# jpreprocess/jbonsai

Hardware: AMD Instinct MI355X
Metric: 48 kHz PCM samples/sec (whole node), batched utterances (higher is better)
Workload: dtype f64

## Files before the change

### jbonsai_amd/csrc/jb_vocoder.hip

```cpp
#include "jb_device.h"

#include <cstdlib>
#include <cstring>

namespace jb {

__global__ void k_pitch(BatchDev bd, VocDev vd)
{
    const int b = blockIdx.y;
    const UttDev *u = bd.utt + b;
    const uint32_t t = blockIdx.x * blockDim.x + threadIdx.x;
    if (t >= u->T)
        return;
    const uint64_t f = u->frame_off + t;
    const double MAX_LF0 = 9.903487552536127, MIN_LF0 = 2.995732273553991;
    auto pitch_of = [&](double l) {
        if (l == kNoData)
            return 0.0;
        const double cl = l < MIN_LF0 ? MIN_LF0 : (l > MAX_LF0 ? MAX_LF0 : l);
        return (double)vd.fs / exp(cl);
    };
    const double p = pitch_of(vd.lf0[f]);
    const double prevp = t > 0 ? pitch_of(vd.lf0[f - 1]) : 0.0;
    vd.pitch[f] = p;
// ... 1157 lines not shown
                    yl = fma(cd[k], d[k], yl);
                const double Y = seg_scan(yl, ks);
                const double Yp = Y * Pl;
                const double v1 = readlane_f64(Yp, 11), v2 = readlane_f64(Yp, 23),
                             v3 = readlane_f64(Yp, 35), v4 = readlane_f64(Yp, 47),
                             v5 = readlane_f64(Yp, 59);
                x += v5;
                x -= v4;
                x += v3;
                x -= v2;
                x += v1;
                double out = v5;
                out += v4;
                out += v3;
                out += v2;
                out += v1;
                ulane = fma(hmask, dpp_f64<DPP_WAVE_SHR1>(Y), l0mask * x);
                x += out;
#pragma unroll
                for (int k = 0; k < TPL; k++)
                    cd[k] += cdinc[k];
                c1 += c1inc;
                ob = (lane == i) ? x * vol : ob;
            }
            if (lane < blen && emit) {
                if (vd.pcm16)
                    vd.pcm16[base * (uint64_t)fp + n0 + (uint64_t)lane] = (int16_t)pcm_i16(ob);
                else
                    vd.pcm[base * (uint64_t)fp + n0 + (uint64_t)lane] = ob;
            }
        }
        (void)ctgt;
    }

    if (wk.save_end)
        save_state(wk.save_end);
}

template <int TPL, int ITEMS>
__global__ __launch_bounds__(128 * ITEMS) void k_vocoder_pair(BatchDev bd, VocDev vd, const VocWork *__restrict__ work,
                                                              uint32_t n_items)
{
    __shared__ double xbuf[ITEMS][2][64];
    __shared__ double obuf[ITEMS][2][64];
    __shared__ uint32_t nblocks_sh[ITEMS];
    const int wv = threadIdx.x >> 6, lane = threadIdx.x & 63;
    const int slot = wv % ITEMS;
    const bool producer = wv >= ITEMS;
    const uint32_t item = blockIdx.x * (uint32_t)ITEMS + (uint32_t)slot;
    const int fp = vd.fperiod, bs = vd.bs, nblk = vd.nblk, nmcp = vd.nmcp;
    VocWork wk{};
    uint32_t t_begin = 0, t_end = 0, t_out = 0;
    int b = 0;
    if (item < n_items) {
        wk = work[item];
        b = (int)wk.utt;
        t_begin = wk.t_start;
        t_out = wk.t_out;
        t_end = min(wk.t_end, bd.utt[b].T);
        if (t_begin >= t_end)
            t_begin = t_end = 0;
    }
    const uint32_t NB = (t_end - t_begin) * (uint32_t)nblk;
    if (!producer && lane == 0)
        nblocks_sh[slot] = NB;
    __syncthreads();
    uint32_t NBmax = 0;
#pragma unroll
    for (int j = 0; j < ITEMS; j++)
        NBmax = max(NBmax, nblocks_sh[j]);
    const uint64_t base = NB ? bd.utt[b].frame_off : 0;
    const double a = wave_uniform(voc_alpha(vd, (uint32_t)b)), iaa = 1.0 - a * a,
                 vol = wave_uniform(voc_volume(vd, (uint32_t)b));
    double *const xb = &xbuf[slot][0][0];
    double *const ob = &obuf[slot][0][0];

    if (producer) {
        double e11[6], e12[6];
#pragma unroll
        for (int i = 0; i < 6; i++)
            e11[i] = e12[i] = 0.0;
        if (NB && wk.load_state) {
#pragma unroll
            for (int i = 0; i < 6; i++) {
                e11[i] = wk.load_state[64 * TPL + 64 + i];
                e12[i] = wk.load_state[64 * TPL + 70 + i];
            }
        }
        auto save_state = [&](double *sp) {
            if (lane == 0) {
#pragma unroll
                for (int i = 0; i < 6; i++) {
                    sp[64 * TPL + 64 + i] = e11[i];
                    sp[64 * TPL + 70 + i] = e12[i];
                }
            }
        };
        uint32_t t = t_begin;
        int q = 0;
        double c1 = 0.0, c1inc = 0.0, gain = 0.0, gq = 0.0;
        for (uint32_t st = 0; st < NBmax + 2; st++) {
            if (st >= 2 && st - 2 < NB) {
                const uint32_t gb = st - 2;
                const uint32_t ts = t_begin + gb / (uint32_t)nblk;
                const int qs = (int)(gb % (uint32_t)nblk), i0 = qs * bs;
                const int blen = min(bs, fp - i0);
                if (ts >= t_out && lane < blen) {
                    const double v = ob[64 * (gb & 1u) + lane] * vol;
                    const uint64_t o = base * (uint64_t)fp + (uint64_t)ts * (uint64_t)fp + (uint64_t)(i0 + lane);
                    if (vd.pcm16)
                        vd.pcm16[o] = (int16_t)pcm_i16(v);
                    else
                        vd.pcm[o] = v;
                }
            }
            if (st < NB) {
                if (q == 0) {
                    if (t == t_out && t_out > t_begin && wk.save_warm)
                        save_state(wk.save_warm);
                    if (t == t_out + vd.ckpt_frames && wk.save_ckpt)
                        save_state(wk.save_ckpt);
                    if (vd.ckpt2_frames && t == t_out + vd.ckpt2_frames && wk.save_ckpt2)
                        save_state(wk.save_ckpt2);
                    const double *bcur = vd.bcoef + (base + t) * (uint64_t)nmcp;
                    const double *bprev =
                        (t > 0) ? bcur - nmcp : (vd.bfirst ? vd.bfirst + (uint64_t)b * (uint64_t)nmcp : bcur);
                    c1 = bprev[1];
                    c1inc = (bcur[1] - c1) / (double)fp;
                    gain = exp(bprev[0]);
                    gq = exp((bcur[0] - bprev[0]) / (double)fp);
                }
                const int i0 = q * bs;
                const int blen = min(bs, fp - i0);
                const double xin = lane < blen ? exc_block_ptr(vd, base, t, exc_code(vd, base, t), q)[i0 + lane] : 0.0;
                double xo = 0.0;
                for (int i = 0; i < blen; i++) {
                    double x = readlane_f64(xin, i) * gain;
                    gain *= gq;
                    double out = 0.0;
#pragma unroll
                    for (int ii = 5; ii >= 1; ii--) {
                        e11[ii] = fma(iaa, e12[ii - 1], a * e11[ii]);
                        e12[ii] = e11[ii] * c1;
                        const double v = e12[ii] * kPPade[ii];
                        x += (ii & 1) ? v : -v;
                        out += v;
                    }
                    e12[0] = x;
                    x += out;
                    c1 += c1inc;
                    xo = (lane == i) ? x : xo;
                }
                if (lane < blen)
                    xb[64 * (st & 1u) + lane] = xo;
                if (++q == nblk) {
                    q = 0;
                    t++;
                }
            }
            __syncthreads();
        }
        if (NB && wk.save_end)
            save_state(wk.save_end);
        return;
    }

    const int M = nmcp - 1;
    const int s = lane / kGroups, g = lane % kGroups;
    const bool active = lane < kPade * kGroups;
    const bool head = active && g == 0;
    const double kappa = ipow(-a, TPL);
    ScanCoef kc, ks;
    {
        const int r16 = lane & 15;
        auto ok = [&](int sh) { return active && g >= sh && r16 >= sh; };
        kc.c1 = ok(1) ? ipow(kappa, 1) : 0.0;
        kc.c2 = ok(2) ? ipow(kappa, 2) : 0.0;
        kc.c4 = ok(4) ? ipow(kappa, 4) : 0.0;
        kc.c8 = ok(8) ? ipow(kappa, 8) : 0.0;
        const int rowstart = lane & ~15, segstart = s * kGroups;
        const bool straddle = active && rowstart > 0 && segstart < rowstart;
        kc.cb = straddle ? ipow(kappa, lane - rowstart + 1) : 0.0;
        ks.c1 = kc.c1 != 0.0 ? 1.0 : 0.0;
        ks.c2 = kc.c2 != 0.0 ? 1.0 : 0.0;
        ks.c4 = kc.c4 != 0.0 ? 1.0 : 0.0;
        ks.c8 = kc.c8 != 0.0 ? 1.0 : 0.0;
        ks.cb = straddle ? 1.0 : 0.0;
    }
    const double nh = (active && !head) ? 1.0 : 0.0;
    const double hmask = (head && s > 0) ? 1.0 : 0.0;
    const double l0mask = (lane == 0) ? 1.0 : 0.0;
    const double Pl = active ? kPPade[s + 1] : 0.0;
    int tapj[TPL];
    bool dotv[TPL];
#pragma unroll
    for (int k = 0; k < TPL; k++) {
        tapj[k] = g * TPL + k + 1;
        dotv[k] = active && tapj[k] >= 2 && tapj[k] <= M;
    }
    double d[TPL], cd[TPL], cdinc[TPL];
#pragma unroll
    for (int k = 0; k < TPL; k++)
        d[k] = cd[k] = cdinc[k] = 0.0;
    double ulane = 0.0;
    if (NB && wk.load_state) {
#pragma unroll
        for (int k = 0; k < TPL; k++)
            d[k] = wk.load_state[64 * k + lane];
        ulane = wk.load_state[64 * TPL + lane];
    }
    auto save_state = [&](double *sp) {
#pragma unroll
        for (int k = 0; k < TPL; k++)
            sp[64 * k + lane] = d[k];
        sp[64 * TPL + lane] = ulane;
    };
    uint32_t t = t_begin;
    int q = 0;
    for (uint32_t st = 0; st < NBmax + 2; st++) {
        if (st >= 1 && st - 1 < NB) {
            const uint32_t gb = st - 1;
            if (q == 0) {
                if (t == t_out && t_out > t_begin && wk.save_warm)
                    save_state(wk.save_warm);
                if (t == t_out + vd.ckpt_frames && wk.save_ckpt)
                    save_state(wk.save_ckpt);
                if (vd.ckpt2_frames && t == t_out + vd.ckpt2_frames && wk.save_ckpt2)
                    save_state(wk.save_ckpt2);
                const double *bcur = vd.bcoef + (base + t) * (uint64_t)nmcp;
                const double *bprev = (t > 0) ? bcur - nmcp : (vd.bfirst ? vd.bfirst + (uint64_t)b * (uint64_t)nmcp : bcur);
#pragma unroll
                for (int k = 0; k < TPL; k++) {
                    const double c0v = dotv[k] ? bprev[tapj[k]] : 0.0;
                    const double c1v = dotv[k] ? bcur[tapj[k]] : 0.0;
                    cd[k] = c0v;
                    cdinc[k] = (c1v - c0v) / (double)fp;
                }
            }
            const int blen = min(bs, fp - q * bs);
            const double *xs = xb + 64 * (gb & 1u);
            double *os = ob + 64 * (gb & 1u);
            double xn = xs[0];
            for (int i = 0; i < blen; i++) {
                double x = xn;
                xn = xs[i + 1 < blen ? i + 1 : i];
                double loc = d[0];
#pragma unroll
                for (int k = 1; k < TPL; k++)
                    loc = fma(-a, loc, d[k]);
                double I = fma(kappa, ulane, loc);
                I = seg_scan(I, kc);
                double r = fma(nh, dpp_f64<DPP_WAVE_SHR1>(I), ulane);
#pragma unroll
                for (int k = 0; k < TPL; k++) {
                    const double rn = fma(-a, r, d[k]);
                    d[k] = fma(a, rn, r);
                    r = rn;
                }
                double yl = cd[0] * d[0];
#pragma unroll
                for (int k = 1; k < TPL; k++)
                    yl = fma(cd[k], d[k], yl);
                const double Y = seg_scan(yl, ks);
                const double Yp = Y * Pl;
                const double v1 = readlane_f64(Yp, 11), v2 = readlane_f64(Yp, 23), v3 = readlane_f64(Yp, 35),
                             v4 = readlane_f64(Yp, 47), v5 = readlane_f64(Yp, 59);
                x += v5;
                x -= v4;
                x += v3;
                x -= v2;
                x += v1;
                double out = v5;
                out += v4;
                out += v3;
                out += v2;
                out += v1;
                ulane = fma(hmask, dpp_f64<DPP_WAVE_SHR1>(Y), l0mask * x);
                x += out;
#pragma unroll
                for (int k = 0; k < TPL; k++)
                    cd[k] += cdinc[k];
                if (lane == 0)
                    os[i] = x;
            }
            if (++q == nblk) {
                q = 0;
                t++;
            }
        }
        __syncthreads();
    }
    if (NB && wk.save_end)
        save_state(wk.save_end);
}

constexpr int DPP_WAVE_SHL1 = 0x130;
constexpr int DPP_ROW_SHL1 = 0x101, DPP_ROW_SHL2 = 0x102, DPP_ROW_SHL4 = 0x104;
__device__ __forceinline__ double fold5(double s)
{
    const double t1 = s + dpp_f64<DPP_ROW_SHL1>(s);
    const double t2 = t1 + dpp_f64<DPP_ROW_SHL2>(t1);
    return t2 + dpp_f64<DPP_ROW_SHL4>(s);
}
constexpr int kLtPf = 4;
constexpr int kLtBalance = 8;
#ifdef JB_LT_STAMPS
constexpr unsigned kLtStampWaves = 4096;
__device__ unsigned long long g_lt_stamp[kLtStampWaves][4];
#endif
#ifdef JB_LT_CLOCKS
__device__ unsigned long long g_lt_clk[8];
#endif

template <int NM, int TPLW_, int kLtWaves, bool EXACT = true, int LPC = 3>
__global__ __launch_bounds__(64 * kLtWaves, 2) void k_vocoder_lt(BatchDev bd, VocDev vd,
                                                       const VocWork *__restrict__ work,
                                                       const uint32_t *__restrict__ order,
                                                       uint32_t n_items)
{
    static_assert(LPC == 3 || LPC == 5, "three lanes x two stage slots, or five lanes x one");
    constexpr int M = NM - 1;
    constexpr int NS = LPC == 3 ? 2 : 1;
    constexpr int kLtChunks = lt_chunks(LPC);
    const int nm = EXACT ? NM : vd.nmcp;
    const int mreal = nm - 1;
    const int TPLW = EXACT ? TPLW_ : (mreal + kGroups - 1) / kGroups;
    const int lane = threadIdx.x % 64;
    const int wv = threadIdx.x / 64;
    const bool idle = LPC == 3 ? lane == 63 : (lane & 15) == 15;
    const int pos = LPC == 3 ? (idle ? 2 : lane % 3) : (idle ? 4 : (lane & 15) % 5);
    const int ci = LPC == 3 ? (idle ? 20 : lane / 3) : (lane >> 4) * 3 + (idle ? 2 : (lane & 15) / 5);
    const uint32_t slot = (blockIdx.x * (uint32_t)kLtWaves + (uint32_t)wv) * (uint32_t)kLtChunks + (uint32_t)ci;
    const uint32_t oslot = (!idle && slot < n_items) ? order[slot] : kLtNoItem;
    const bool has = oslot != kLtNoItem;
    const bool lead = has && pos == 0;
    const uint32_t item = has ? oslot : 0u;
    struct {
        uint32_t utt, t_start, t_out, t_end;
        const double *load_state;
    } wk = {0, 0, 0, 0, nullptr};
    if (has) {
        const VocWork &w0 = work[item];
        wk.utt = w0.utt;
        wk.t_start = w0.t_start;
        wk.t_out = w0.t_out;
        wk.t_end = w0.t_end;
        wk.load_state = w0.load_state;
    }
    const uint32_t T = has ? bd.utt[wk.utt].T : 0;
    if (wk.t_end > T)
        wk.t_end = T;
    const uint32_t nfr = wk.t_end > wk.t_start ? wk.t_end - wk.t_start : 0;
    uint32_t maxfr = nfr;
    for (int o = 32; o > 0; o >>= 1)
        maxfr = max(maxfr, (uint32_t)__shfl_xor((int)maxfr, o));
    __shared__ uint32_t prog[8];
    if (kLtWaves == 8 && lane == 0)
        prog[wv] = maxfr == 0 ? 0xffffffffu : 0u;
    if (maxfr == 0)
        return;
#ifdef JB_LT_STAMPS
    const unsigned stamp_w = blockIdx.x * (unsigned)kLtWaves + (unsigned)wv;
    if (lane == 0 && stamp_w < kLtStampWaves) {
        unsigned hw, xcc;
        asm volatile("s_getreg_b32 %0, hwreg(HW_REG_HW_ID)" : "=s"(hw));
        asm volatile("s_getreg_b32 %0, hwreg(HW_REG_XCC_ID, 0, 4)" : "=s"(xcc));
        g_lt_stamp[stamp_w][0] = wall_clock64();
        g_lt_stamp[stamp_w][2] = (unsigned long long)hw | ((unsigned long long)xcc << 32);
        g_lt_stamp[stamp_w][3] = maxfr;
    }
#endif
#ifdef JB_LT_CLOCKS
    const int clk_slot = wv != 0 ? -1 : blockIdx.x == 0 ? 0 : blockIdx.x == gridDim.x / 2 ? 4 : -1;
    if (clk_slot >= 0 && lane == 0) {
        g_lt_clk[clk_slot] = clock64();
        g_lt_clk[clk_slot + 1] = wall_clock64();
    }
#endif
    const uint64_t base = has ? bd.utt[wk.utt].frame_off : 0;
    const int fp = vd.fperiod;
    double a = vd.alpha, vol = vd.volume;
    if (vd.uvoc) {
        const uint32_t u0 = wave_uniform(wk.utt);
        a = wave_uniform(vd.uvoc[u0].alpha);
        vol = wave_uniform(vd.uvoc[u0].volume);
    }
    const double na = -a, iaa = 1.0 - a * a;
    const int s0 = NS * pos;
    const double w0 = kPPade[s0 + 1];
    const double w1 = (NS == 2 && s0 + 1 < kPade) ? kPPade[s0 + 2] : 0.0;
    const double wa = (NS == 1 && (pos & 1)) ? -w0 : w0;

    __shared__ double2 cc_[kLtWaves][NM - 1][kLtChunks];
    __shared__ double gqs_[kLtWaves][kLtChunks];
    double2 (*const cc)[kLtChunks] = cc_[wv];
    double *const gqs = gqs_[wv];
#define JB_LT_FENCE() asm volatile("s_waitcnt lgkmcnt(0)" ::: "memory")

    if (!EXACT && has)
        for (int k = nm + pos; k < NM; k += LPC)
            cc[k - 1][ci] = make_double2(0.0, 0.0);
    double d[NS][M + 1];
    double u[NS];
    double gain = 1.0;
    double e11[NS], e12[NS], ein = 0.0;
#pragma unroll
    for (int q = 0; q < NS; q++) {
        e11[q] = e12[q] = 0.0;
        u[q] = 0.0;
#pragma unroll
        for (int j = 0; j <= M; j++)
            d[q][j] = 0.0;
    }

    auto layout_tpl = [&]() {
        int tp = TPLW;
        if (!EXACT)
            asm volatile("" : "+s"(tp));
        return tp;
    };
    if (wk.load_state) {
        const double *sp = wk.load_state;
        const int tpl = layout_tpl();
#pragma unroll
        for (int q = 0; q < NS; q++) {
            const int st = s0 + q;
            if (st < kPade) {
                u[q] = sp[64 * tpl + kGroups * st];
                int kk = 0, gg = 0;
#pragma unroll
                for (int j = 1; j <= M; j++) {
                    if (EXACT)
                        d[q][j] = sp[64 * ((j - 1) % TPLW_) + kGroups * st + (j - 1) / TPLW_];
                    else if (j <= mreal)
                        d[q][j] = sp[64 * kk + kGroups * st + gg];
                    if (++kk == tpl) {
                        kk = 0;
                        gg++;
                    }
                }
            }
        }
#pragma unroll
        for (int q = 0; q < NS; q++) {
            const int st = s0 + 1 + q;
            if (st <= kPade) {
                e11[q] = sp[64 * tpl + 64 + st];
                e12[q] = sp[64 * tpl + 70 + st];
            }
        }
        ein = sp[64 * tpl + 70 + s0];
    }
    auto save_state = [&](double *sp) {
        const int tpl = layout_tpl();
#pragma unroll
        for (int q = 0; q < NS; q++) {
            const int st = s0 + q;
            if (st < kPade) {
                sp[64 * tpl + kGroups * st] = u[q];
                int kk = 0, gg = 0;
#pragma unroll
                for (int j = 1; j <= M; j++) {
                    if (EXACT)
                        sp[64 * ((j - 1) % TPLW_) + kGroups * st + (j - 1) / TPLW_] = d[q][j];
                    else if (j <= mreal)
                        sp[64 * kk + kGroups * st + gg] = d[q][j];
                    if (++kk == tpl) {
                        kk = 0;
                        gg++;
                    }
                }
            }
        }
#pragma unroll
        for (int q = 0; q < NS; q++) {
            const int st = s0 + 1 + q;
            if (st <= kPade) {
                sp[64 * tpl + 64 + st] = e11[q];
                sp[64 * tpl + 70 + st] = e12[q];
            }
        }
        if (pos == 0) {
            sp[64 * tpl + 64] = 0.0;
            sp[64 * tpl + 70] = ein;
        }
    };

    for (uint32_t tl = 0; tl < maxfr; tl++) {
        const bool act = tl < nfr;
        const uint32_t t = wk.t_start + (act ? tl : 0);
        const uint64_t f = base + t;
        const bool emit = act && lead && t >= wk.t_out;
        if (act && t == wk.t_out && wk.t_out > wk.t_start) {
            double *sw_ = work[item].save_warm;
            if (sw_)
                save_state(sw_);
        }
        if (act && t == wk.t_out + vd.ckpt_frames) {
            double *sc_ = work[item].save_ckpt;
            if (sc_)
                save_state(sc_);
        }
        if (act && vd.ckpt2_frames && t == wk.t_out + vd.ckpt2_frames) {
            double *sc_ = work[item].save_ckpt2;
            if (sc_)
                save_state(sc_);
        }
        JB_LT_FENCE();
        if (has) {
            const double *bcur = vd.bcoef + f * (uint64_t)nm;
            const double *bprev = (t > 0) ? bcur - nm : (vd.bfirst ? vd.bfirst + (uint64_t)wk.utt * nm : bcur);
            for (int k = 1 + pos; k < nm; k += LPC) {
                const double c0v = bprev[k], c1v = bcur[k];
                cc[k - 1][ci] = make_double2(c0v, (c1v - c0v) / (double)fp);
            }
            gain = exp(bprev[0]);
            if (pos == 0)
                gqs[ci] = exp((bcur[0] - bprev[0]) / (double)fp);
        }
        JB_LT_FENCE();
        const uint32_t xcode = act ? exc_code(vd, base, t) : 1u;
        const int xbs = vd.bs;
        auto xblock = [&](int q) -> const double * { return act ? exc_block_ptr(vd, base, t, xcode, q) : vd.noise; };
        const double *xq = xblock(0);
        double *op = vd.pcm + (base + t) * (uint64_t)fp;
        double xn = act ? xq[0] : 0.0;
        const double gq = gqs[ci];
        double oA = 0.0, oB = 0.0;
        auto put_pair = [&](int at) {
            if (vd.pcm16)
                *reinterpret_cast<uint32_t *>(vd.pcm16 + (base + t) * (uint64_t)fp + at) = pcm_i16x2(oA, oB);
            else
                *reinterpret_cast<double2 *>(op + at) = make_double2(oA, oB);
        };
        double xo;
        {
            const int n1 = fp > 1 ? 1 : 0;
            asm volatile("global_load_dwordx2 %0, %1, off" : "=v"(xo) : "v"(xq + n1) : "memory");
        }
        auto sample = [&](const int i, auto ODDC) {
            constexpr bool ODD = decltype(ODDC)::value;
            double x;
            if (ODD) {
                asm volatile("s_waitcnt vmcnt(0)" : "+v"(xo)::"memory");
                x = xo * gain;
            } else {
                asm volatile("s_waitcnt vmcnt(1)" : "+v"(xn)::"memory");
                x = xn * gain;
            }
            gain *= gq;
            if (!ODD && i > 0 && emit)
                put_pair(i - 2);
            {
                const int nx = i + 2 < fp ? i + 2 : fp - 1;
                if (ODD)
                    asm volatile("global_load_dwordx2 %0, %1, off" : "=v"(xo) : "v"(xq + nx) : "memory");
                else
                    asm volatile("global_load_dwordx2 %0, %1, off" : "=v"(xn) : "v"(xq + nx) : "memory");
            }
            const double fi = (double)i;
            double db1;
            {
                const double2 c1p = cc[0][ci];
                const double c1 = fma(fi, c1p.y, c1p.x);
                if constexpr (NS == 2) {
                    e11[1] = fma(iaa, e12[0], a * e11[1]);
                    e11[0] = fma(iaa, ein, a * e11[0]);
                    e12[1] = e11[1] * c1;
                    e12[0] = e11[0] * c1;
                    const double dv1 = w1 * e12[1];
                    const double da = fma(w0, e12[0], -dv1);
                    db1 = fma(w0, e12[0], dv1);
                    x += da + dpp_f64<DPP_WAVE_SHL1>(da + dpp_f64<DPP_WAVE_SHL1>(da));
                } else {
                    e11[0] = fma(iaa, ein, a * e11[0]);
                    e12[0] = e11[0] * c1;
                    db1 = w0 * e12[0];
                    x += fold5(wa * e12[0]);
                }
                const double eprev = dpp_f64<DPP_WAVE_SHR1>(e12[NS - 1]);
                ein = pos == 0 ? x : eprev;
            }
            double r[NS], y[NS];
#pragma unroll
            for (int q = 0; q < NS; q++)
                r[q] = u[q];
            static_assert(M >= 2, "the dot products start at tap 2");
            typedef double v2d __attribute__((ext_vector_type(2)));
            v2d cq[kLtPf];
            const uint32_t cca = (uint32_t)(uintptr_t)&cc[0][ci];
#define JB_LDS_RD(dst, tapj)                                                                     \
    asm volatile("ds_read_b128 %0, %1 offset:%2"                                                 \
                 : "=v"(dst)                                                                     \
                 : "v"(cca), "n"(((tapj)-1) * (int)(sizeof(double2) * kLtChunks)))
#pragma unroll
            for (int k = 0; k < kLtPf; k++)
                JB_LDS_RD(cq[k], 2 + k);
            static_assert(kLtPf == 4 && M % 2 == 0 && M >= 6, "pair schedule: four slots, taps 2..M in pairs + one");
            double cv[M + 2];
            auto wait_pair = [&](const int j, const int younger) {
                v2d &qa = cq[(j - 2) % kLtPf], &qb = cq[(j - 1) % kLtPf];
                switch (younger) {
                case 0: asm volatile("s_waitcnt lgkmcnt(0)" : "+v"(qa), "+v"(qb)); break;
                case 1: asm volatile("s_waitcnt lgkmcnt(1)" : "+v"(qa), "+v"(qb)); break;
                default: asm volatile("s_waitcnt lgkmcnt(2)" : "+v"(qa), "+v"(qb)); break;
                }
            };
            cv[1] = 0.0;
#pragma unroll
            for (int j = 1; j <= M; j++) {
                if (j == 1)
                    wait_pair(2, 2);
                else if (j % 2 == 0 && j + 2 <= M)
                    wait_pair(j + 2, j + 4 <= M ? 1 : 0);
                if (j + 1 <= M) {
                    const int sq = (j - 1) % kLtPf;
                    cv[j + 1] = fma(fi, cq[sq].y, cq[sq].x);
                    if (j + 5 <= M)
                        JB_LDS_RD(cq[sq], j + 5);
                }
                const double cj = cv[j];
                if constexpr (NS == 1) {
                    double rn0;
                    if (j <= 2) {
                        asm volatile("v_fma_f64 %[rn0], %[na], %[r0], %[d0]\n\t"
                            "v_fma_f64 %[d0], %[a], %[rn0], %[r0]"
                            : [rn0] "=&v"(rn0), [d0] "+v"(d[0][j])
                            : [na] "s"(na), [a] "s"(a), [r0] "v"(r[0]));
                    } else if (j == 3) {
                        asm volatile("v_fma_f64 %[rn0], %[na], %[r0], %[d0]\n\t"
                            "v_mul_f64 %[y0], %[c], %[dp]\n\t"
                            "v_fma_f64 %[d0], %[a], %[rn0], %[r0]"
                            : [rn0] "=&v"(rn0), [d0] "+v"(d[0][j]), [y0] "=&v"(y[0])
                            : [na] "s"(na), [a] "s"(a), [r0] "v"(r[0]), [c] "v"(cv[j - 1]), [dp] "v"(d[0][j - 1]));
                    } else {
                        asm volatile("v_fma_f64 %[rn0], %[na], %[r0], %[d0]\n\t"
                            "v_fma_f64 %[y0], %[c], %[dp], %[y0]\n\t"
                            "v_fma_f64 %[d0], %[a], %[rn0], %[r0]"
                            : [rn0] "=&v"(rn0), [d0] "+v"(d[0][j]), [y0] "+v"(y[0])
                            : [na] "s"(na), [a] "s"(a), [r0] "v"(r[0]), [c] "v"(cv[j - 1]), [dp] "v"(d[0][j - 1]));
                    }
                    r[0] = rn0;
                    if (j == M)
                        y[0] = fma(cj, d[0][M], y[0]);
                } else {
                    double rn0, rn1;
                    if (j == 2) {
                        asm volatile("v_fma_f64 %[rn0], %[na], %[r0], %[d0]\n\t"
                            "v_fma_f64 %[rn1], %[na], %[r1], %[d1]\n\t"
                            "v_fma_f64 %[d0], %[a], %[rn0], %[r0]\n\t"
                            "v_fma_f64 %[d1], %[a], %[rn1], %[r1]\n\t"
                            "v_mul_f64 %[y0], %[c], %[d0]\n\t"
                            "v_mul_f64 %[y1], %[c], %[d1]"
                            : [rn0] "=&v"(rn0), [rn1] "=&v"(rn1), [d0] "+v"(d[0][j]), [d1] "+v"(d[1][j]),
                              [y0] "=&v"(y[0]), [y1] "=&v"(y[1])
                            : [na] "s"(na), [a] "s"(a), [r0] "v"(r[0]), [r1] "v"(r[1]), [c] "v"(cj));
                    } else if (j > 2) {
                        asm volatile("v_fma_f64 %[rn0], %[na], %[r0], %[d0]\n\t"
                            "v_fma_f64 %[rn1], %[na], %[r1], %[d1]\n\t"
                            "v_fma_f64 %[d0], %[a], %[rn0], %[r0]\n\t"
                            "v_fma_f64 %[d1], %[a], %[rn1], %[r1]\n\t"
                            "v_fma_f64 %[y0], %[c], %[d0], %[y0]\n\t"
                            "v_fma_f64 %[y1], %[c], %[d1], %[y1]"
                            : [rn0] "=&v"(rn0), [rn1] "=&v"(rn1), [d0] "+v"(d[0][j]), [d1] "+v"(d[1][j]),
                              [y0] "+v"(y[0]), [y1] "+v"(y[1])
                            : [na] "s"(na), [a] "s"(a), [r0] "v"(r[0]), [r1] "v"(r[1]), [c] "v"(cj));
                    } else {
                        asm volatile("v_fma_f64 %[rn0], %[na], %[r0], %[d0]\n\t"
                            "v_fma_f64 %[rn1], %[na], %[r1], %[d1]\n\t"
                            "v_fma_f64 %[d0], %[a], %[rn0], %[r0]\n\t"
                            "v_fma_f64 %[d1], %[a], %[rn1], %[r1]"
                            : [rn0] "=&v"(rn0), [rn1] "=&v"(rn1), [d0] "+v"(d[0][j]), [d1] "+v"(d[1][j])
                            : [na] "s"(na), [a] "s"(a), [r0] "v"(r[0]), [r1] "v"(r[1]));
                    }
                    r[0] = rn0;
                    r[1] = rn1;
                }
            }
#undef JB_LDS_RD
            double ssum, psum;
            if constexpr (NS == 2) {
                const double v1 = w1 * y[1];
                const double sb = fma(w0, y[0], v1), sa = fma(w0, y[0], db1 - v1);
                ssum = sa + dpp_f64<DPP_WAVE_SHL1>(sa + dpp_f64<DPP_WAVE_SHL1>(sa));
                psum = sb + dpp_f64<DPP_WAVE_SHL1>(sb + dpp_f64<DPP_WAVE_SHL1>(sb));
            } else {
                ssum = fold5(fma(wa, y[0], db1));
                psum = fold5(w0 * y[0]);
            }
            const double yprev = dpp_f64<DPP_WAVE_SHR1>(y[NS - 1]);
            const double xmid = x + ssum;
            x = xmid + psum;
            if constexpr (NS == 2)
                u[1] = y[0];
            u[0] = pos == 0 ? xmid : yprev;
            const double pv = x * vol;
            if (ODD)
                oB = pv;
            else
                oA = pv;
        };
        int xnext = xbs, xqn = 1;
        for (int i2 = 0; i2 < fp; i2 += 2) {
            if (i2 + 2 == xnext && xnext < fp) {
                xq = xblock(xqn);
                xqn++;
                xnext += xbs;
            }
            if (kLtWaves == 8 && i2 % kLtBalance == 0) {
                const uint32_t mine = tl * (uint32_t)fp + (uint32_t)i2;
                uint32_t theirs;
                asm volatile("ds_write_b32 %1, %2\n\t"
                             "ds_read_b32 %0, %3\n\t"
                             "s_waitcnt lgkmcnt(0)"
                             : "=v"(theirs)
                             : "v"((uint32_t)(uintptr_t)&prog[wv]), "v"(mine), "v"((uint32_t)(uintptr_t)&prog[wv ^ 4])
                             : "memory");
                if (mine > (uint32_t)__builtin_amdgcn_readfirstlane((int)theirs))
                    __builtin_amdgcn_s_setprio(0);
                else
                    __builtin_amdgcn_s_setprio(1);
            }
            sample(i2, std::false_type{});
            sample(i2 + 1, std::true_type{});
        }
        asm volatile("s_waitcnt vmcnt(0)" : "+v"(xn), "+v"(xo)::"memory");
        if (emit)
            put_pair(fp - 2);
        if (act && tl + 1 == nfr) {
            double *se_ = work[item].save_end;
            if (se_)
                save_state(se_);
        }
    }
    if (kLtWaves == 8 && lane == 0)
        prog[wv] = 0xffffffffu;
#ifdef JB_LT_STAMPS
    if (lane == 0 && stamp_w < kLtStampWaves)
        g_lt_stamp[stamp_w][1] = wall_clock64();
#endif
#ifdef JB_LT_CLOCKS
    if (clk_slot >= 0 && lane == 0) {
        g_lt_clk[clk_slot + 2] = clock64();
        g_lt_clk[clk_slot + 3] = wall_clock64();
    }
#endif
}

__device__ __forceinline__ bool voc_state_differs(const double *__restrict__ a, const double *__restrict__ r,
                                                  int nfilt, int ntaps, double tol, int lane, double *md_out,
                                                  double *mr_out)
{
    double md = 0.0, mr = 0.0;
    const int urow = nfilt - 76;
    const int tpl = urow / 64;
    for (int k = lane; k < nfilt; k += 64) {
        if (ntaps < 0) {
        } else if (k < urow) {
            const int ln = k & 63, kk = k >> 6;
            if (ln >= kGroups * kPade || (ln % kGroups) * tpl + kk >= ntaps)
                continue;
        } else if (k < urow + 64 && ((k - urow) % kGroups != 0 || (k - urow) >= kGroups * kPade)) {
            continue;
        }
        const double x = a[k], y = r[k];
        md = fmax(md, fabs(x - y));
        mr = fmax(mr, fabs(y));
        if (!(x == x) || !(y == y))
            md = 1e300;
    }
    for (int o = 32; o > 0; o >>= 1) {
        md = fmax(md, __shfl_xor(md, o));
        mr = fmax(mr, __shfl_xor(mr, o));
    }
    *md_out = md;
    *mr_out = mr;
    return md > tol * mr && md > 1e-300;
}

__global__ __launch_bounds__(64) void k_voc_verify(const VocWork *__restrict__ work, uint32_t n_items,
                                                    int nfilt , int ntaps, double tol,
                                                    uint8_t *bad, uint32_t *n_bad)
{
    const uint32_t i = blockIdx.x;
    if (i >= n_items)
        return;
    const VocWork wk = work[i];
    const int lane = threadIdx.x;
    if (!wk.save_warm || i == 0) {
        if (lane == 0)
            bad[i] = 0;
        return;
    }
    double md, mr;
    const bool isbad = voc_state_differs(wk.save_warm, work[i - 1].save_end, nfilt, ntaps, tol, lane, &md, &mr);
    if (lane == 0) {
        bad[i] = isbad;
        if (isbad)
            atomicAdd(n_bad, 1u);
#ifdef JB_VERIFY_DEBUG
        if (isbad)
            printf("handoff item %u utt %u t_out %u: max|diff| %.3e max|state| %.3e ratio %.3e\n", i, wk.utt,
                   wk.t_out, md, mr, md / mr);
#endif
    }
}

__global__ __launch_bounds__(64) void k_voc_verify_pairs(const double *const *__restrict__ pairs, uint32_t n_pairs,
                                                          int nfilt, int ntaps, double tol, uint8_t *bad,
                                                          uint32_t *n_bad)
{
    const uint32_t i = blockIdx.x;
    if (i >= n_pairs)
        return;
    const int lane = threadIdx.x;
    double md, mr;
    const bool isbad = voc_state_differs(pairs[2 * i], pairs[2 * i + 1], nfilt, ntaps, tol, lane, &md, &mr);
    if (lane == 0) {
        bad[i] = isbad;
        if (isbad)
            atomicAdd(n_bad, 1u);
#ifdef JB_VERIFY_DEBUG
        printf("state pair %u: max|diff| %.3e max|state| %.3e %s\n", i, md, mr, isbad ? "FAIL" : "ok");
#endif
    }
}

static int tpl_for(int nmcp)
{
    int M = nmcp - 1;
    int tpl = (M + kGroups - 1) / kGroups;
    return tpl < 1 ? 1 : tpl;
}

int vocoder_state_doubles(int nmcp) { return voc_state_doubles(tpl_for(nmcp)); }

hipError_t launch_pitch(const BatchDev &bd, const VocDev &vd, hipStream_t stream)
{
    if (bd.B == 0 || bd.maxT == 0)
        return hipSuccess;
    dim3 grid((bd.maxT + 255) / 256, bd.B), block(256);
    hipLaunchKernelGGL(k_pitch, grid, block, 0, stream, bd, vd);
    return hipGetLastError();
}

hipError_t launch_mc2b(const BatchDev &bd, const VocDev &vd, hipStream_t stream)
{
    if (bd.B == 0 || bd.maxT == 0)
        return hipSuccess;
    dim3 grid((bd.maxT + kMc2bFrames - 1) / kMc2bFrames, bd.B), block(kMc2bFrames);
    hipLaunchKernelGGL(k_mc2b, grid, block, 0, stream, bd, vd);
    return hipGetLastError();
}

static int current_device_cus()
{
    static int cus_of[64] = {0};
    int dev = 0, cus = 0;
    if (hipGetDevice(&dev) != hipSuccess || dev < 0 || dev >= 64)
        return 0;
    if ((cus = cus_of[dev]) == 0) {
        if (hipDeviceGetAttribute(&cus, hipDeviceAttributeMultiprocessorCount, dev) != hipSuccess || cus <= 0)
            return 0;
        cus_of[dev] = cus;
    }
    return cus;
}

bool excite_is_split(const VocDev &vd)
{
    return vd.fperiod % kExw == 0 && vd.fperiod <= 256 && vd.fperiod >= kExwHalo && (vd.nlpf == 31 || vd.nlpf == 15) &&
           vd.nblk <= 4 && vd.fperiod % vd.bs == 0;
}

hipError_t launch_excite_noise(const BatchDev &bd, const VocDev &vd, hipStream_t stream)
{
    if (bd.B == 0 || bd.maxT == 0 || !excite_is_split(vd))
        return hipSuccess;
    if (!vd.exc_src || !vd.exc_gen || !vd.exc_gen_count || !vd.exc_tab)
        return hipErrorInvalidValue;
    hipError_t e = hipMemsetAsync(vd.exc_gen_count, 0, sizeof(uint32_t), stream);
    if (e != hipSuccess)
        return e;
    const dim3 block(256);
    const dim3 gcls((bd.maxT + 255) / 256, bd.B), gtab((bd.maxT + 3) / 4);
    constexpr size_t pad = 32 * 1024;
    int cus = current_device_cus();
    if (cus <= 0)
        cus = 256;
    const dim3 ggen((unsigned)(3 * cus));
    if (vd.nlpf == 31) {
        hipLaunchKernelGGL(k_exc_classify<31>, gcls, block, 0, stream, bd, vd);
        if (!vd.exc_no_table)
            hipLaunchKernelGGL(k_exc_table<31>, gtab, block, 0, stream, bd, vd);
        JB_DBG_SKIP_IF(4, hipLaunchKernelGGL(k_exc_general<31>, ggen, block, pad, stream, bd, vd));
    } else {
        hipLaunchKernelGGL(k_exc_classify<15>, gcls, block, 0, stream, bd, vd);
        if (!vd.exc_no_table)
            hipLaunchKernelGGL(k_exc_table<15>, gtab, block, 0, stream, bd, vd);
        hipLaunchKernelGGL(k_exc_general<15>, ggen, block, pad, stream, bd, vd);
    }
    return hipGetLastError();
}

hipError_t launch_excite(const BatchDev &bd, const VocDev &vd, hipStream_t stream)
{
    if (bd.B == 0 || bd.maxT == 0)
        return hipSuccess;
    if (excite_is_split(vd)) {
        dim3 gfix((bd.maxT + 4 * kFixFrames - 1) / (4 * kFixFrames), bd.B), block(256);
        if (vd.nlpf == 31)
            JB_DBG_SKIP_IF(8, hipLaunchKernelGGL(k_excite_fix<31>, gfix, block, 0, stream, bd, vd));
        else
            hipLaunchKernelGGL(k_excite_fix<15>, gfix, block, 0, stream, bd, vd);
        return hipGetLastError();
    }
    const uint64_t maxN = (uint64_t)bd.maxT * (uint64_t)vd.fperiod;
    dim3 grid((unsigned)((maxN + kExcBlock - 1) / kExcBlock), bd.B), block(kExcBlock);
    if (vd.nlpf == 0) {
        if (!vd.uv_before)
            return hipErrorInvalidValue;
        hipLaunchKernelGGL(k_uv_scan, dim3(bd.B), dim3(64), 0, stream, bd, vd);
        hipLaunchKernelGGL(k_excite_nolpf, grid, block, 0, stream, bd, vd);
        return hipGetLastError();
    }
    if (excite_fits_staged(vd))
        hipLaunchKernelGGL(k_excite, grid, block, 0, stream, bd, vd);
    else
        hipLaunchKernelGGL(k_excite_any, grid, block, (size_t)(kExcBlock + vd.nlpf - 1) * sizeof(double), stream, bd, vd);
    return hipGetLastError();
}

constexpr unsigned kPulseQueueWaves = 512;
hipError_t launch_pulse(const BatchDev &bd, const VocDev &vd, hipStream_t stream)
{
    if (bd.B == 0 || bd.maxT == 0)
        return hipSuccess;
    hipLaunchKernelGGL(k_run_scan, dim3(1), dim3(256), 0, stream, bd, vd);
    JB_DBG_SKIP_IF(64, hipLaunchKernelGGL(k_pulse_queue, dim3(kPulseQueueWaves), dim3(64), 0, stream, bd, vd));
    return hipGetLastError();
}

hipError_t launch_voc_verify(const VocWork *work_dev, uint32_t n_items, int state_doubles, int ntaps, double tol,
                             uint8_t *bad, uint32_t *n_bad, hipStream_t stream)
{
    if (n_items == 0)
        return hipSuccess;
    hipLaunchKernelGGL(k_voc_verify, dim3(n_items), dim3(64), 0, stream, work_dev, n_items,
                       ntaps < 0 ? state_doubles : state_doubles - 4, ntaps, tol, bad, n_bad);
    return hipGetLastError();
}

hipError_t launch_voc_verify_pairs(const double *const *pairs_dev, uint32_t n_pairs, int state_doubles, int ntaps,
                                   double tol, uint8_t *bad, uint32_t *n_bad, hipStream_t stream)
{
    if (n_pairs == 0)
        return hipSuccess;
    hipLaunchKernelGGL(k_voc_verify_pairs, dim3(n_pairs), dim3(64), 0, stream, pairs_dev, n_pairs,
                       ntaps < 0 ? state_doubles : state_doubles - 4, ntaps, tol, bad, n_bad);
    return hipGetLastError();
}

hipError_t launch_vocoder_ls(const BatchDev &bd, const VocDev &vd, const VocWork *work_dev,
                             const uint32_t *order_dev, uint32_t n_items, int waves_per_simd, hipStream_t stream)
{
    if (n_items == 0)
        return hipSuccess;
    if ((waves_per_simd != 1 && waves_per_simd != 2) || !vocoder_ls_supported(vd.nmcp))
        return hipErrorInvalidValue;
    const int wv = 4 * waves_per_simd;
    const int code = lt_code_nm(vd.nmcp);
    const bool exact = vd.nmcp == 35 || vd.nmcp == 25;
    const uint32_t per_wg = (uint32_t)(vocoder_ls_chunks_per_wave(vd.nmcp) * wv);
    dim3 grid((n_items + per_wg - 1) / per_wg), block(64 * wv);
#define JB_LT_LAUNCH(NMc, TPLc, EX, LPCc)                                                                              \
    do {                                                                                                           \
        if (wv == 8)                                                                                               \
            hipLaunchKernelGGL((k_vocoder_lt<NMc, TPLc, 8, EX, LPCc>), grid, block, 0, stream, bd, vd, work_dev,      \
                               order_dev, n_items);                                                                \
        else                                                                                                       \
            hipLaunchKernelGGL((k_vocoder_lt<NMc, TPLc, 4, EX, LPCc>), grid, block, 0, stream, bd, vd, work_dev,      \
                               order_dev, n_items);                                                                \
    } while (0)
    if (exact && code == 35)
        JB_LT_LAUNCH(35, 3, true, 3);
    else if (exact && code == 25)
        JB_LT_LAUNCH(25, 2, true, 3);
    else if (code == 25)
        JB_LT_LAUNCH(25, 2, false, 3);
    else if (code == 31)
        JB_LT_LAUNCH(31, 3, false, 3);
    else if (code == 35)
        JB_LT_LAUNCH(35, 3, false, 3);
    else if (code == 41)
        JB_LT_LAUNCH(41, 4, false, 5);
    else if (code == 51)
        JB_LT_LAUNCH(51, 5, false, 5);
    else
        JB_LT_LAUNCH(61, 5, false, 5);
#undef JB_LT_LAUNCH
#ifdef JB_LT_STAMPS
    if (const char *path = getenv("JB_LT_STAMPS_FILE")) {
        static unsigned long long st[kLtStampWaves][4];
        hipStreamSynchronize(stream);
        const unsigned nw = std::min<unsigned>(kLtStampWaves, grid.x * (unsigned)wv);
        if (hipMemcpyFromSymbol(st, HIP_SYMBOL(g_lt_stamp), sizeof st) == hipSuccess)
            if (FILE *f = fopen(path, "w")) {
                fprintf(f, "# wave start_10ns end_10ns hw_id xcc frames   (k_vocoder_lt, %u waves, %d per workgroup)\n", nw, wv);
                for (unsigned w = 0; w < nw; w++)
                    fprintf(f, "%u %llu %llu %llu %llu %llu\n", w, st[w][0], st[w][1], st[w][2] & 0xffffffffull,
                            st[w][2] >> 32, st[w][3]);
                fclose(f);
            }
        unsigned long long t0 = ~0ull, last[16] = {0};
        for (unsigned w = 0; w < nw; w++)
            if (st[w][0] && st[w][0] < t0)
                t0 = st[w][0];
        for (unsigned w = 0; w < nw; w++)
            last[(st[w][2] >> 32) & 15] = std::max(last[(st[w][2] >> 32) & 15], st[w][1]);
        fprintf(stderr, "k_vocoder_lt last wave end per XCD, ms:");
        for (int x = 0; x < 8; x++)
            fprintf(stderr, " %.2f", last[x] ? (double)(last[x] - t0) / 1e5 : 0.0);
        fprintf(stderr, "\n");
    }
#endif
#ifdef JB_LT_CLOCKS
    {
        unsigned long long c[8];
        hipStreamSynchronize(stream);
        if (hipMemcpyFromSymbol(c, HIP_SYMBOL(g_lt_clk), sizeof c) == hipSuccess)
            for (int k = 0; k < 8; k += 4) {
                const double us = (double)(c[k + 3] - c[k + 1]) / 100.0;
                fprintf(stderr, "k_vocoder_lt wave %d: %.3f ms, %.0f shader-clock ticks = %.3f GHz\n", k / 4, us / 1e3,
                        (double)(c[k + 2] - c[k]), (double)(c[k + 2] - c[k]) / us / 1e3);
            }
    }
#endif
// ... 78 lines not shown
```

Baseline: 20.26 billion.

## Defer cross-lane output reductions via ds_bpermute to overlap with next sample

For the two-stage-per-lane layout, the cross-lane shifts for the input-side sum, the post-filter sum and the previous-lane state are moved from DPP to asynchronous ds_bpermute LDS ops. The final output combine is deferred into the next sample, where it is waited on alongside other LDS reads, so the latency sits off the serial dependency chain. The output pointer is also advanced incrementally instead of being recomputed per pair. The risk is more LDS traffic and extra register pressure from the carried partial values, plus subtle ordering hazards in the pipelined recurrence.

```diff
diff --git a/jbonsai_amd/csrc/jb_vocoder.hip b/jbonsai_amd/csrc/jb_vocoder.hip
--- a/jbonsai_amd/csrc/jb_vocoder.hip
+++ b/jbonsai_amd/csrc/jb_vocoder.hip
@@ -1483,6 +1483,10 @@
     const double t2 = t1 + dpp_f64<DPP_ROW_SHL2>(t1);
     return t2 + dpp_f64<DPP_ROW_SHL4>(s);
 }
+struct LtXd {
+    int lo, hi;
+};
+__device__ __forceinline__ double lt_xd(const LtXd &v) { return __hiloint2double(v.hi, v.lo); }
 constexpr int kLtPf = 4;
 constexpr int kLtBalance = 8;
 #ifdef JB_LT_STAMPS
@@ -1632,6 +1636,11 @@
         }
         ein = sp[64 * tpl + 70 + s0];
     }
+    [[maybe_unused]] const uint32_t bpa = (uint32_t)lane * 4u;
+#define JB_BPERM(dst, src, off) \
+    asm volatile("ds_bpermute_b32 %0, %1, %2 offset:%3" : "=v"(dst) : "v"(bpa), "v"(src), "n"(off))
+    [[maybe_unused]] double xmid_c = u[0], sb_c = 0.0;
+    [[maybe_unused]] LtXd yp_c = {__double2loint(u[0]), __double2hiint(u[0])}, p1_c = {0, 0}, p2_c = {0, 0};
     auto save_state = [&](double *sp) {
         const int tpl = layout_tpl();
 #pragma unroll
@@ -1704,23 +1713,35 @@
         const int xbs = vd.bs;
         auto xblock = [&](int q) -> const double * { return act ? exc_block_ptr(vd, base, t, xcode, q) : vd.noise; };
         const double *xq = xblock(0);
-        double *op = vd.pcm + (base + t) * (uint64_t)fp;
+        const int64_t pstep = vd.pcm16 ? 4 : 16;
+        char *pq = vd.pcm16 ? reinterpret_cast<char *>(vd.pcm16 + (base + t) * (uint64_t)fp)
+                            : reinterpret_cast<char *>(vd.pcm + (base + t) * (uint64_t)fp);
         double xn = act ? xq[0] : 0.0;
         const double gq = gqs[ci];
         double oA = 0.0, oB = 0.0;
-        auto put_pair = [&](int at) {
+        auto put_pair = [&](auto BACK) {
+            constexpr int back = decltype(BACK)::value;
             if (vd.pcm16)
-                *reinterpret_cast<uint32_t *>(vd.pcm16 + (base + t) * (uint64_t)fp + at) = pcm_i16x2(oA, oB);
+                *reinterpret_cast<uint32_t *>(pq - back * 4) = pcm_i16x2(oA, oB);
             else
-                *reinterpret_cast<double2 *>(op + at) = make_double2(oA, oB);
+                *reinterpret_cast<double2 *>(pq - back * 16) = make_double2(oA, oB);
         };
         double xo;
         {
             const int n1 = fp > 1 ? 1 : 0;
             asm volatile("global_load_dwordx2 %0, %1, off" : "=v"(xo) : "v"(xq + n1) : "memory");
         }
+        typedef double v2d __attribute__((ext_vector_type(2)));
+        const uint32_t cca = (uint32_t)(uintptr_t)&cc[0][ci];
+        [[maybe_unused]] auto collect = [&](double &o) {
+            u[0] = pos == 0 ? xmid_c : lt_xd(yp_c);
+            o = (xmid_c + (sb_c + (lt_xd(p1_c) + lt_xd(p2_c)))) * vol;
+        };
         auto sample = [&](const int i, auto ODDC) {
             constexpr bool ODD = decltype(ODDC)::value;
+            v2d c1q;
+            if constexpr (NS == 2)
+                asm volatile("ds_read_b128 %0, %1" : "=v"(c1q) : "v"(cca));
             double x;
             if (ODD) {
                 asm volatile("s_waitcnt vmcnt(0)" : "+v"(xo)::"memory");
@@ -1730,8 +1751,17 @@
                 x = xn * gain;
             }
             gain *= gq;
-            if (!ODD && i > 0 && emit)
-                put_pair(i - 2);
+            if constexpr (NS == 2) {
+                asm volatile("s_waitcnt lgkmcnt(0)"
+                             : "+v"(c1q), "+v"(yp_c.lo), "+v"(yp_c.hi), "+v"(p1_c.lo), "+v"(p1_c.hi), "+v"(p2_c.lo),
+                               "+v"(p2_c.hi));
+                collect(ODD ? oA : oB);
+            }
+            if (!ODD) {
+                pq += pstep;
+                if (i > 0 && emit)
+                    put_pair(std::integral_constant<int, 2>{});
+            }
             {
                 const int nx = i + 2 < fp ? i + 2 : fp - 1;
                 if (ODD)
@@ -1741,25 +1771,33 @@
             }
             const double fi = (double)i;
             double db1;
-            {
+            [[maybe_unused]] double da;
+            [[maybe_unused]] LtXd d1, d2, ep;
+            if constexpr (NS == 2) {
+                const double c1 = fma(fi, c1q.y, c1q.x);
+                e11[1] = fma(iaa, e12[0], a * e11[1]);
+                e11[0] = fma(iaa, ein, a * e11[0]);
+                e12[1] = e11[1] * c1;
+                e12[0] = e11[0] * c1;
+                const double dv1 = w1 * e12[1];
+                da = fma(w0, e12[0], -dv1);
+                db1 = fma(w0, e12[0], dv1);
+                const int dal = __double2loint(da), dah = __double2hiint(da);
+                const int epl = __double2loint(e12[1]), eph = __double2hiint(e12[1]);
+                JB_BPERM(d1.lo, dal, 4);
+                JB_BPERM(d1.hi, dah, 4);
+                JB_BPERM(d2.lo, dal, 8);
+                JB_BPERM(d2.hi, dah, 8);
+                JB_BPERM(ep.lo, epl, 252);
+                JB_BPERM(ep.hi, eph, 252);
+            } else {
                 const double2 c1p = cc[0][ci];
                 const double c1 = fma(fi, c1p.y, c1p.x);
-                if constexpr (NS == 2) {
-                    e11[1] = fma(iaa, e12[0], a * e11[1]);
-                    e11[0] = fma(iaa, ein, a * e11[0]);
-                    e12[1] = e11[1] * c1;
-                    e12[0] = e11[0] * c1;
-                    const double dv1 = w1 * e12[1];
-                    const double da = fma(w0, e12[0], -dv1);
-                    db1 = fma(w0, e12[0], dv1);
-                    x += da + dpp_f64<DPP_WAVE_SHL1>(da + dpp_f64<DPP_WAVE_SHL1>(da));
-                } else {
-                    e11[0] = fma(iaa, ein, a * e11[0]);
-                    e12[0] = e11[0] * c1;
-                    db1 = w0 * e12[0];
-                    x += fold5(wa * e12[0]);
-                }
-                const double eprev = dpp_f64<DPP_WAVE_SHR1>(e12[NS - 1]);
+                e11[0] = fma(iaa, ein, a * e11[0]);
+                e12[0] = e11[0] * c1;
+                db1 = w0 * e12[0];
+                x += fold5(wa * e12[0]);
+                const double eprev = dpp_f64<DPP_WAVE_SHR1>(e12[0]);
                 ein = pos == 0 ? x : eprev;
             }
             double r[NS], y[NS];
@@ -1767,9 +1805,7 @@
             for (int q = 0; q < NS; q++)
                 r[q] = u[q];
             static_assert(M >= 2, "the dot products start at tap 2");
-            typedef double v2d __attribute__((ext_vector_type(2)));
             v2d cq[kLtPf];
-            const uint32_t cca = (uint32_t)(uintptr_t)&cc[0][ci];
 #define JB_LDS_RD(dst, tapj)                                                                     \
     asm volatile("ds_read_b128 %0, %1 offset:%2"                                                 \
                  : "=v"(dst)                                                                     \
@@ -1790,9 +1826,17 @@
             cv[1] = 0.0;
 #pragma unroll
             for (int j = 1; j <= M; j++) {
-                if (j == 1)
-                    wait_pair(2, 2);
-                else if (j % 2 == 0 && j + 2 <= M)
+                if (j == 1) {
+                    if constexpr (NS == 2) {
+                        asm volatile("s_waitcnt lgkmcnt(2)"
+                                     : "+v"(cq[0]), "+v"(cq[1]), "+v"(d1.lo), "+v"(d1.hi), "+v"(d2.lo), "+v"(d2.hi),
+                                       "+v"(ep.lo), "+v"(ep.hi));
+                        x += da + (lt_xd(d1) + lt_xd(d2));
+                        ein = pos == 0 ? x : lt_xd(ep);
+                    } else {
+                        wait_pair(2, 2);
+                    }
+                } else if (j % 2 == 0 && j + 2 <= M)
                     wait_pair(j + 2, j + 4 <= M ? 1 : 0);
                 if (j + 1 <= M) {
                     const int sq = (j - 1) % kLtPf;
@@ -1859,27 +1903,34 @@
                 }
             }
 #undef JB_LDS_RD
-            double ssum, psum;
             if constexpr (NS == 2) {
                 const double v1 = w1 * y[1];
                 const double sb = fma(w0, y[0], v1), sa = fma(w0, y[0], db1 - v1);
-                ssum = sa + dpp_f64<DPP_WAVE_SHL1>(sa + dpp_f64<DPP_WAVE_SHL1>(sa));
-                psum = sb + dpp_f64<DPP_WAVE_SHL1>(sb + dpp_f64<DPP_WAVE_SHL1>(sb));
+                const double ssum = sa + dpp_f64<DPP_WAVE_SHL1>(sa + dpp_f64<DPP_WAVE_SHL1>(sa));
+                const int sbl = __double2loint(sb), sbh = __double2hiint(sb);
+                const int ypl = __double2loint(y[1]), yph = __double2hiint(y[1]);
+                JB_BPERM(p1_c.lo, sbl, 4);
+                JB_BPERM(p1_c.hi, sbh, 4);
+                JB_BPERM(p2_c.lo, sbl, 8);
+                JB_BPERM(p2_c.hi, sbh, 8);
+                JB_BPERM(yp_c.lo, ypl, 252);
+                JB_BPERM(yp_c.hi, yph, 252);
+                xmid_c = x + ssum;
+                sb_c = sb;
+                u[1] = y[0];
             } else {
-                ssum = fold5(fma(wa, y[0], db1));
-                psum = fold5(w0 * y[0]);
-            }
-            const double yprev = dpp_f64<DPP_WAVE_SHR1>(y[NS - 1]);
-            const double xmid = x + ssum;
-            x = xmid + psum;
-            if constexpr (NS == 2)
-                u[1] = y[0];
-            u[0] = pos == 0 ? xmid : yprev;
-            const double pv = x * vol;
-            if (ODD)
-                oB = pv;
-            else
-                oA = pv;
+                const double ssum = fold5(fma(wa, y[0], db1));
+                const double psum = fold5(w0 * y[0]);
+                const double yprev = dpp_f64<DPP_WAVE_SHR1>(y[0]);
+                const double xmid = x + ssum;
+                x = xmid + psum;
+                u[0] = pos == 0 ? xmid : yprev;
+                const double pv = x * vol;
+                if (ODD)
+                    oB = pv;
+                else
+                    oA = pv;
+            }
         };
         int xnext = xbs, xqn = 1;
         for (int i2 = 0; i2 < fp; i2 += 2) {
@@ -1906,14 +1957,24 @@
             sample(i2 + 1, std::true_type{});
         }
         asm volatile("s_waitcnt vmcnt(0)" : "+v"(xn), "+v"(xo)::"memory");
+        if constexpr (NS == 2) {
+            asm volatile("s_waitcnt lgkmcnt(0)"
+                         : "+v"(yp_c.lo), "+v"(yp_c.hi), "+v"(p1_c.lo), "+v"(p1_c.hi), "+v"(p2_c.lo), "+v"(p2_c.hi));
+            collect(oB);
+            xmid_c = u[0];
+            yp_c = {__double2loint(u[0]), __double2hiint(u[0])};
+            sb_c = 0.0;
+            p1_c = p2_c = {0, 0};
+        }
         if (emit)
-            put_pair(fp - 2);
+            put_pair(std::integral_constant<int, 1>{});
         if (act && tl + 1 == nfr) {
             double *se_ = work[item].save_end;
             if (se_)
                 save_state(se_);
         }
     }
+#undef JB_BPERM
     if (kLtWaves == 8 && lane == 0)
         prog[wv] = 0xffffffffu;
 #ifdef JB_LT_STAMPS
```

After: 19.78 billion. 0.976x the previous value.
